# atosystem/SpeechCLIP

Hardware: AMD Instinct MI355X
Metric: speech-image pairs/sec/node (Parallel SpeechCLIP base) (higher is better)
Workload: dtype bf16; 1 GPU; Parallel SpeechCLIP base (HuBERT-base + ViT-B/32) forward + InfoNCE, 10 s/16 kHz audio + 224^2 images; pairs_per_gpu=256, global_batch=256, audio_samples=160000, frames=499, parallelism=single, weights=random-init (no network), mode=forward + loss

## Files before the change

include/speechclip_hip.h:

```cpp
#ifndef SPEECHCLIP_HIP_H
#define SPEECHCLIP_HIP_H

#include <stdint.h>

#ifdef __cplusplus
extern "C" {
#endif

int sc_abi_version(void);
const char* sc_last_error(void);

#define SC_ACT_NONE 0
#define SC_ACT_GELU 1
#define SC_ACT_QUICKGELU 2
#define SC_GEMM_ACT_MASK 0x3
#define SC_GEMM_OUT_F32 0x10
#define SC_GEMM_F16 0x20
#define SC_GEMM_RES_AFTER_ACT 0x0

int sc_gemm_bf16(const void* A, int64_t lda, const void* W, int64_t ldw, void* C, int64_t ldc,
                 const float* bias, const void* residual, int64_t ldr,
                 int64_t M, int N, int K, int flags, void* stream);
int sc_set_gemm_workspace(void* workspace, int64_t bytes);
int sc_gemm_last_path(void);
int sc_debug_vendor_stream_slot(void* stream);

int sc_gemm_bf16_batched(const void* A, int64_t lda, int64_t strideA, const void* W, int64_t ldw,
                         int64_t strideW, int w_mod, void* C, int64_t ldc, int64_t strideC,
                         const float* bias, int64_t M, int N, int K, int batch, int flags, void* stream);
int sc_gemm_bf16_batched2(const void* A, int64_t lda, int64_t strideA, int64_t strideA2, const void* W, int64_t ldw, int64_t strideW, int64_t strideW2,
                          void* C, int64_t ldc, int64_t strideC, int64_t strideC2, int64_t M, int N, int K, int outer, int inner, int flags, void* stream);

#define SC_LN_IN_F32 0x1
#define SC_LN_OUT_F32 0x2
#define SC_LN_GELU 0x4
#define SC_LN_OUT_F16 0x8
int sc_layernorm(const void* x, int64_t ld_in, const float* gamma, const float* beta, void* out, int64_t ld_out,
                 int64_t rows, int D, float eps, int flags, void* stream);

#define SC_WS_NORMALIZE 0x1
#define SC_WS_IN_F32 0x2
int sc_weighted_sum_fwd(const void* hidden, int64_t layer_stride, const float* weights, void* out, int n_layers,
                        int64_t rows, int D, int flags, float eps, void* stream);

#define SC_L2NORM_IN_F32 0x1
#define SC_L2NORM_CLAMP 0x2
int sc_l2norm_fwd(const void* x, int64_t ld_in, float* out, int64_t rows, int D, int flags, void* stream);

int sc_hidden_normalize(void* hidden, int in_f32, int n_layers, int B, int Tp, int T, int D, int method, float* workspace, void* stream);

int sc_splitk_reduce_f32(const float* partials, int nsplit, int64_t M, int N, const float* bias, const float* residual, int64_t ldr, float* out, int act,
                         void* stream);

int sc_wave_layernorm(const float* wav, float* out, const int32_t* lens, int B, int64_t ld, float eps, void* stream);

#define SC_ATTN_CAUSAL 0x1
#define SC_ATTN_F16 0x2
int sc_attention_fwd(const void* q, const void* k, const void* v, void* out, const int32_t* klens, int B, int H,
                     int T, int head_dim, int64_t ld_qkv, int64_t ld_out, float scale, int flags, void* stream);

int sc_attention_fwd_dropout(const void* q, const void* k, const void* v, void* out, const int32_t* klens, int B, int H, int T, int head_dim,
                             int64_t ld_qkv, int64_t ld_out, float scale, int causal, float drop_p, uint32_t seed, void* stream);
int sc_dropout_bf16(const void* x, const void* residual, void* out, int64_t n, float drop_p, uint32_t seed, void* stream);
int sc_dropout_add_layernorm_bf16(const void* x, const void* residual, const float* gamma, const float* beta, void* out, int64_t rows, int D, float eps,
                                  float drop_p, uint32_t seed, void* stream);

int sc_cls_attention_fwd(const void* cls_qkv, const void* kv_x, int64_t ld_kv, const int32_t* lens, void* out, int B, int T,
                         int NQ, int H, int head_dim, float scale, void* stream);

#define SC_ATTN_HD_OUT_F32 0x10
int sc_attention_hd_fwd(const void* q, const void* k, const void* v, void* out, const int32_t* klens, int B, int H, int Tq, int Tk,
                        int head_dim, int64_t q_bs, int64_t q_rs, int64_t kv_bs, int64_t kv_rs, int64_t o_bs, int64_t o_rs,
                        float scale, float drop_p, uint32_t seed, int flags, void* stream);

int sc_attention_rows_fwd(const void* q, const void* k, const void* v, void* out, const uint8_t* key_padding_mask, int B, int H, int L,
                          int head_dim, int64_t ld_qkv, int64_t ld_out, float scale, void* stream);

int sc_attention_probs_fwd(const void* q, const void* k, float* probs, const uint8_t* key_padding_mask, int B, int H, int L, int head_dim,
                           int n_rows, int64_t ld_qkv, float scale, void* stream);

int sc_topk_rows_f32(const float* x, int64_t ld, int64_t rows, int V, int K, float* vals, int32_t* idx, void* stream);

int sc_cls_pool_fwd(const void* x, int64_t ld_x, const void* cls_tok, const float* scores, const float* cls_scores,
                    const int32_t* lens, void* xbar, int B, int T, int NQ, int R, int D, void* stream);
int sc_cls_pool_fwd_split(const void* x, int64_t ld_x, const void* cls_tok, const float* scores, const float* cls_scores,
                          const int32_t* lens, void* xbar_hilo, int B, int T, int NQ, int R, int D, int nblk, void* stream);

int64_t sc_conv0_stats_workspace_bytes(int B);
int sc_conv0_gn_coef(const float* wav, int64_t ld, const float* w, const float* gamma, const float* beta, void* workspace,
                     float* coef, int B, int C, int T0, float eps, void* stream);
int64_t sc_conv0_wfrag_workspace_bytes(int B);
int sc_conv0_fwd(const float* wav, int64_t ld, int64_t L, const float* w, const float* bias, const float* coef, void* out, int B,
                 int C, int T0, int P, int mode, void* wfrag_ws, void* stream);

int sc_posconv_conv(const void* x, const int32_t* valid, const void* wg, void* conv, int B, int Tp, int D, int G, int Kw, void* stream);
int sc_posconv_pack(const void* x, const int32_t* valid, void* xg, int B, int Tp, int D, int G, int Kw, void* stream);
int sc_posconv_finish(const void* x, const int32_t* valid, const void* conv, const float* bias, const float* gamma, const float* beta,
                      void* out, int B, int Tp, int D, int G, int out_f32, float eps, void* stream);

int sc_crop_pad(const float* wav, int64_t ld, const int32_t* starts, const int32_t* lens, float* out, int B, int Lout, void* stream);

int sc_image_normalize_u8(const void* u8_hwc, float* out_chw, int B, int H, int W, const float* mean3, const float* std3, void* stream);
int sc_vit_patchify(const float* img, void* cols, int B, int R, int p, int Kpad, void* stream);
int sc_vit_embed(const void* patch, const float* cls, const float* pos, const float* gamma, const float* beta, float* out, int B,
                 int ntok, int D, float eps, void* stream);

int64_t sc_infonce_workspace_bytes(int Bg);
int sc_infonce_fwd(const float* feat_a, const float* feat_b, const int64_t* ids, void* workspace, float* out3, int Bg, int E,
                   float inv_temperature, float margin, int dcl, int a2b, int b2a, void* stream);

int sc_kw_affine(const float* x, const float* scale, const float* shift, float* out, int64_t rows, int K, int D, void* stream);
int64_t sc_cosine_workspace_bytes(int R, int V);
int sc_cosine_scores(const float* a, const float* emb, void* workspace, float* out, int R, int V, int E, float eps, void* stream);
int sc_cosine_refine(float* scores, const float* a, const float* emb, int R, int V, int E, float delta, float eps, void* stream);
int64_t sc_vq_workspace_bytes(int R, int V);
int sc_vq_fwd(const float* scores, int64_t* targets, float* stats2, float* ent_per_t, void* workspace, int R, int K, int V,
              const int32_t* host_mask_ids, int n_mask, void* stream);
int sc_gather_rows(const float* src, const int64_t* idx, float* out, int R, int E, void* stream);
int sc_retrieval_ranks(const float* score, int64_t ld, const int64_t* own_ids, const int64_t* cand_ids, int32_t* rank, int n, int m, void* stream);

int sc_sgemm(int transa, int transb, int M, int N, int K, float alpha, const float* A, int64_t lda, const float* B, int64_t ldb, float beta,
             float* C, int64_t ldc, const float* bias, void* stream);
int sc_sgemm_batched(int transa, int transb, int M, int N, int K, float alpha, const float* A, int64_t lda, int64_t strideA, const float* B,
                     int64_t ldb, int64_t strideB, float beta, float* C, int64_t ldc, int64_t strideC, const float* bias, int64_t strideBias,
                     int batch, void* stream);
int sc_cls_pool_train_fwd(const void* x, int64_t ld_x, const float* cls_tok, const float* scores, const float* cls_scores,
                          const int32_t* lens, float* p_out, float* xbar, int B, int T, int NQ, int R, int D, float drop_p, uint32_t seed,
                          void* stream);
int sc_cls_pool_bwd(const void* x, int64_t ld_x, const float* cls_tok, const void* hidden, int hidden_f32, int64_t layer_stride, int n_layers,
                    int normalize,
                    const float* p, const float* dzbar, const float* u, const int32_t* lens, float* ds_ws, float* pp_ws, float* du,
                    float* dcls_key, float* dalpha, int B, int T, int NQ, int R, int D, int nsplit, float drop_p, uint32_t seed, void* stream);
int sc_layernorm_bwd(const float* x, const float* dy, const float* gamma, float* dx, float* dgamma, float* dbeta, float* stats_ws, int rows,
                     int D, float eps, int accumulate_dx, void* stream);
int sc_gelu_f32(const float* z, float* y_or_dh, int64_t n, int backward, void* stream);
int sc_colsum(const float* x, int64_t ld, int rows, int cols, float* out, int accumulate, void* stream);
int sc_l2norm_bwd(const float* x, const float* dy, float* dx, int rows, int D, void* stream);
int sc_dropout_f32(const float* x, float* y, int64_t n, float drop_p, uint32_t seed, void* stream);
int sc_add_rows_f32(const float* a, const float* b, float* out, int rows, int cols, int b_rows, float alpha, void* stream);
int sc_mix_softmax_bwd(const float* w, const float* dalpha_b, int B, int n, float* dw, void* stream);
int sc_split_hilo_bf16(const float* a, int64_t lda, void* out, int64_t M, int K, int nblk, void* stream);
int sc_attn_small_bwd(const void* qkv, const float* dout, float* dqkv, int B, int L, int heads, int head_dim, int causal, void* stream);
int sc_quickgelu_f32(const float* z, void* y_or_dh, int64_t n, int backward, int out_bf16, void* stream);
int sc_vq_st_bwd(const float* cos_scores, float* dprob_inout, float* rowdot, int R, int V, float temp, const int* mask_ids, int n_mask, void* stream);
int sc_cosine_bwd_finish(const float* a, const float* G, const float* rowdot, float* da, int R, int E, float eps, void* stream);
int sc_kw_bn_train_fwd(const float* x, const float* gamma, const float* beta, float* y, float* mean_out, float* rstd_out, float* running_mean,
                       float* running_var, int B, int K, int E, float momentum, float eps, void* stream);
int sc_kw_bn_bwd(const float* x, const float* dy, const float* gamma, const float* mean, const float* rstd, float* dx, float* dgamma, float* dbeta,
                 int B, int K, int E, void* stream);
int64_t sc_infonce_bwd_workspace_bytes(int Bg);
int sc_infonce_bwd(const float* feat_a, const float* feat_b, const int64_t* ids, const void* fwd_workspace, void* bwd_workspace, float* G,
// ... 59 lines not shown
```

speechclip_amd/_lib.py:

```python
import ctypes
import os
from ctypes import c_char_p, c_float, c_int, c_int64, c_uint32, c_void_p

import torch

_HERE = os.path.dirname(os.path.abspath(__file__))
LIB_PATH = os.environ.get("SPEECHCLIP_HIP_LIB") or os.path.join(_HERE, "libspeechclip_hip.so")

ACT_NONE, ACT_GELU, ACT_QUICKGELU = 0, 1, 2
GEMM_OUT_F32 = 0x10
GEMM_F16 = 0x20
ATTN_CAUSAL, ATTN_F16 = 0x1, 0x2
ATTN_HD_OUT_F32 = 0x10

_lib = None


class SpeechClipHipError(RuntimeError):
    pass


def lib():
    global _lib
    if _lib is None:
        if not os.path.exists(LIB_PATH):
            raise SpeechClipHipError(
                f"{LIB_PATH} not found: build it with `python -c 'import __graft_entry__ as g; g.build()'` "
                "(make -C speechclip_amd/csrc).  There is no CPU/PyTorch fallback for the hot path.")
        _lib = ctypes.CDLL(LIB_PATH)
        _lib.sc_last_error.restype = c_char_p
        _declare(_lib)
        mode = os.environ.get("SC_GEMM_KERNEL_MODE")
        if mode:
            try:
                _lib.sc_debug_set_gemm_mode(int(mode))
            except ValueError:
                import warnings
                warnings.warn(f"SC_GEMM_KERNEL_MODE={mode!r} is not an integer: ignored")
    return _lib


def _declare(L):
    P, I, L64, F, U32 = c_void_p, c_int, c_int64, c_float, c_uint32
    sigs = {
        "sc_abi_version": ([], c_int),
        "sc_set_gemm_workspace": ([P, L64], c_int),
        "sc_gemm_bf16": ([P, L64, P, L64, P, L64, P, P, L64, L64, I, I, I, P], c_int),
        "sc_gemm_bf16_batched": ([P, L64, L64, P, L64, L64, I, P, L64, L64, P, L64, I, I, I, I, P], c_int),
        "sc_layernorm": ([P, L64, P, P, P, L64, L64, I, F, I, P], c_int),
        "sc_weighted_sum_fwd": ([P, L64, P, P, I, L64, I, I, F, P], c_int),
        "sc_transpose_bf16": ([P, L64, L64, P, L64, L64, I, I, I, I, P], c_int),
        "sc_attn_softmax_bwd": ([P, P, L64, L64, P, L64, P, L64, L64, P, P, P, I, I, I, F, P], c_int),
        "sc_attn_softmax_bwd_dropout": ([P, P, L64, L64, P, L64, P, L64, L64, P, P, P, I, I, I, F, F, U32, I, I, P], c_int),
        "sc_attn_softmax_bwd_heads": ([P, P, L64, L64, P, L64, P, L64, L64, P, P, P, I, I, I, I, F, F, U32, P], c_int),
        "sc_attn_bwd_probs": ([P, P, P, L64, P, P, L64, P, P, P, I, I, I, I, F, F, U32, P], c_int),
        "sc_gemm_bf16_batched2": ([P, L64, L64, L64, P, L64, L64, L64, P, L64, L64, L64, L64, I, I, I, I, I, P], c_int),
        "sc_gelu_bwd_bf16": ([P, P, P, L64, P], c_int),
        "sc_layernorm_bwd_bf16_partials": ([L64], c_int64),
        "sc_layernorm_bwd_bf16": ([P, P, P, P, P, L64, I, F, P], c_int),
        "sc_colsum_bf16_workspace_bytes": ([L64, I], c_int64),
        "sc_colsum_bf16": ([P, L64, L64, I, P, P, I, P], c_int),
        "sc_axpy_bf16": ([P, P, F, L64, P], c_int),
        "sc_cls_pool_dz": ([P, P, P, P, P, P, I, I, I, I, I, L64, P], c_int),
        "sc_l2norm_fwd": ([P, L64, P, L64, I, I, P], c_int),
        "sc_splitk_reduce_f32": ([P, I, L64, I, P, P, L64, P, I, P], c_int),
        "sc_hidden_normalize": ([P, I, I, I, I, I, I, I, P, P], c_int),
        "sc_wave_layernorm": ([P, P, P, I, L64, F, P], c_int),
        "sc_attention_fwd": ([P, P, P, P, P, I, I, I, I, L64, L64, F, I, P], c_int),
        "sc_attention_fwd_dropout": ([P, P, P, P, P, I, I, I, I, L64, L64, F, I, F, U32, P], c_int),
        "sc_attention_hd_fwd": ([P, P, P, P, P, I, I, I, I, I, L64, L64, L64, L64, L64, L64, F, F, U32, I, P], c_int),
        "sc_dropout_bf16": ([P, P, P, L64, F, U32, P], c_int),
        "sc_dropout_add_layernorm_bf16": ([P, P, P, P, P, L64, I, F, F, U32, P], c_int),
        "sc_cls_attention_fwd": ([P, P, L64, P, P, I, I, I, I, I, F, P], c_int),
        "sc_attention_rows_fwd": ([P, P, P, P, P, I, I, I, I, L64, L64, F, P], c_int),
        "sc_attention_probs_fwd": ([P, P, P, P, I, I, I, I, I, L64, F, P], c_int),
        "sc_posconv_finish_train": ([P, P, P, P, P, P, I, I, I, I, P], c_int),
        "sc_posconv_dgrad_finish": ([P, P, P, P, I, I, I, I, P], c_int),
        "sc_reverse_rows_bf16": ([P, P, I, I, I, P], c_int),
        "sc_conv0_bwd": ([P, L64, P, P, P, P, P, I, I, I, I, F, P], c_int),
        "sc_conv0_wgrad": ([P, L64, P, P, I, I, I, I, P], c_int),
        "sc_topk_rows_f32": ([P, L64, L64, I, I, P, P, P], c_int),
        "sc_cls_pool_fwd": ([P, L64, P, P, P, P, P, I, I, I, I, I, P], c_int),
        "sc_cls_pool_fwd_split": ([P, L64, P, P, P, P, P, I, I, I, I, I, I, P], c_int),
        "sc_conv0_stats_workspace_bytes": ([I], c_int64),
        "sc_conv0_gn_coef": ([P, L64, P, P, P, P, P, I, I, I, F, P], c_int),
        "sc_conv0_wfrag_workspace_bytes": ([I], c_int64),
        "sc_conv0_fwd": ([P, L64, L64, P, P, P, P, I, I, I, I, I, P, P], c_int),
        "sc_posconv_conv": ([P, P, P, P, I, I, I, I, I, P], c_int),
        "sc_posconv_pack": ([P, P, P, I, I, I, I, I, P], c_int),
        "sc_posconv_finish": ([P, P, P, P, P, P, P, I, I, I, I, I, F, P], c_int),
        "sc_crop_pad": ([P, L64, P, P, P, I, I, P], c_int),
        "sc_conv0_fwd_packed": ([P, L64, L64, P, P, P, P, I, I, I, P, I, I, I, P, P], c_int),
        "sc_posconv_conv_packed": ([P, P, P, P, P, I, I, I, I, I, P], c_int),
        "sc_posconv_finish_packed": ([P, P, P, P, P, P, P, P, I, L64, I, I, I, F, P], c_int),
        "sc_attention_fwd_packed": ([P, P, P, P, P, P, I, I, I, L64, I, L64, L64, F, F, U32, I, P], c_int),
        "sc_unpack_rows": ([P, L64, P, P, L64, I, I, I, I, I, P], c_int),
        "sc_pack_rows": ([P, L64, P, P, L64, I, I, I, L64, I, I, P], c_int),
        "sc_attention_bwd_packed_workspace_bytes": ([L64, I], c_int64),
        "sc_attention_bwd_packed": ([P, P, P, L64, P, P, L64, P, P, I, I, I, L64, I, F, F, U32, P, P, P, L64, P, P], c_int),
        "sc_image_normalize_u8": ([P, P, I, I, I, P, P, P], c_int),
        "sc_vit_patchify": ([P, P, I, I, I, I, P], c_int),
        "sc_vit_embed": ([P, P, P, P, P, P, I, I, I, F, P], c_int),
        "sc_infonce_workspace_bytes": ([I], c_int64),
        "sc_infonce_fwd": ([P, P, P, P, P, I, I, F, F, I, I, I, P], c_int),
        "sc_kw_affine": ([P, P, P, P, L64, I, I, P], c_int),
        "sc_cosine_workspace_bytes": ([I, I], c_int64),
        "sc_cosine_scores": ([P, P, P, P, I, I, I, F, P], c_int),
        "sc_vq_workspace_bytes": ([I, I], c_int64),
        "sc_vq_fwd": ([P, P, P, P, P, I, I, I, P, I, P], c_int),
        "sc_gather_rows": ([P, P, P, I, I, P], c_int),
        "sc_retrieval_ranks": ([P, L64, P, P, P, I, I, P], c_int),
        "sc_sgemm": ([I, I, I, I, I, F, P, L64, P, L64, F, P, L64, P, P], c_int),
        "sc_sgemm_batched": ([I, I, I, I, I, F, P, L64, L64, P, L64, L64, F, P, L64, L64, P, L64, I, P], c_int),
        "sc_cls_pool_train_fwd": ([P, L64, P, P, P, P, P, P, I, I, I, I, I, F, U32, P], c_int),
        "sc_cls_pool_bwd": ([P, L64, P, P, I, L64, I, I, P, P, P, P, P, P, P, P, P, I, I, I, I, I, I, F, U32, P], c_int),
        "sc_layernorm_bwd": ([P, P, P, P, P, P, P, I, I, F, I, P], c_int),
        "sc_gelu_f32": ([P, P, L64, I, P], c_int),
        "sc_gemm_last_path": ([], c_int),
        "sc_debug_set_gemm_mode": ([I], None),
        "sc_debug_poison_gemm_sched": ([], c_int),
        "sc_debug_vendor_stream_slot": ([P], c_int),
        "sc_split_hilo_bf16": ([P, L64, P, L64, I, I, P], c_int),
        "sc_cosine_refine": ([P, P, P, I, I, I, F, F, P], c_int),
        "sc_attn_small_bwd": ([P, P, P, I, I, I, I, I, P], c_int),
        "sc_quickgelu_f32": ([P, P, L64, I, I, P], c_int),
        "sc_vq_st_bwd": ([P, P, P, I, I, F, P, I, P], c_int),
        "sc_cosine_bwd_finish": ([P, P, P, P, I, I, F, P], c_int),
        "sc_kw_bn_train_fwd": ([P, P, P, P, P, P, P, P, I, I, I, F, F, P], c_int),
        "sc_kw_bn_bwd": ([P, P, P, P, P, P, P, P, I, I, I, P], c_int),
        "sc_colsum": ([P, L64, I, I, P, I, P], c_int),
        "sc_l2norm_bwd": ([P, P, P, I, I, P], c_int),
        "sc_dropout_f32": ([P, P, L64, F, U32, P], c_int),
        "sc_mix_softmax_bwd": ([P, P, I, I, P, P], c_int),
        "sc_add_rows_f32": ([P, P, P, I, I, I, F, P], c_int),
        "sc_infonce_bwd_workspace_bytes": ([I], c_int64),
        "sc_infonce_bwd": ([P, P, P, P, P, P, P, I, I, F, F, I, I, I, P], c_int),
        "sc_grad_norm_workspace_bytes": ([], c_int64),
        "sc_grad_norm": ([P, L64, F, P, P, P], c_int),
        "sc_adam_step": ([P, P, P, P, L64, P, F, F, F, F, F, I, P], c_int),
    }
    for name, (args, res) in sigs.items():
        fn = getattr(L, name)
        fn.argtypes = args
        fn.restype = res


def check(rc, what):
    if rc != 0:
        raise SpeechClipHipError(f"{what} failed (rc={rc}): {lib().sc_last_error().decode()}")


def ptr(t):
    return 0 if t is None else t.data_ptr()


def stream():
# ... 9 lines not shown
```

speechclip_amd/csrc/attention_rows.hip:

```cpp
#include "common.h"
#include "../../include/speechclip_hip.h"

namespace {

constexpr int ROWS_PER_BLOCK = 4;
constexpr int MAX_HD = 1024;

__global__ __launch_bounds__(256) void attention_rows_kernel(const bf16_t* __restrict__ q, const bf16_t* __restrict__ k, const bf16_t* __restrict__ v,
                                                             bf16_t* __restrict__ out, const uint8_t* __restrict__ pad, int B, int H, int L, int hd,
                                                             int64_t ld_qkv, int64_t ld_out, float scale_log2e) {
    extern __shared__ float sq[];
    const int lane = threadIdx.x & 63, wave = threadIdx.x >> 6;
    const int qblocks = (L + ROWS_PER_BLOCK - 1) / ROWS_PER_BLOCK;
    const int bh = blockIdx.x / qblocks, qb = blockIdx.x - bh * qblocks;
    const int b = bh / H, h = bh - b * H;
    const int i = qb * ROWS_PER_BLOCK + wave;
    if (i >= L) return;
    float* myq = sq + wave * hd;
    const bf16_t* qrow = q + ((int64_t)b * L + i) * ld_qkv + h * hd;
    for (int d = lane; d < hd; d += 64) myq[d] = bf2f(qrow[d]) * scale_log2e;
    __builtin_amdgcn_wave_barrier();
    asm volatile("s_waitcnt lgkmcnt(0)" ::: "memory");
    const int nd = (hd + 63) / 64;
    float acc[MAX_HD / 64];
#pragma unroll
    for (int m = 0; m < MAX_HD / 64; ++m) acc[m] = 0.f;
    float run_max = -INFINITY, run_sum = 0.f;
    const uint8_t* prow = pad ? pad + (int64_t)b * L : nullptr;
    for (int j0 = 0; j0 < L; j0 += 64) {
        const int j = j0 + lane;
        const bool valid = j < L && !(prow && prow[j]);
        float s = -INFINITY;
        if (valid) {
            const bf16_t* krow = k + ((int64_t)b * L + j) * ld_qkv + h * hd;
            float dot = 0.f;
            int d = 0;
            for (; d + 8 <= hd; d += 8) {
                const uint4 kk = *(const uint4*)(krow + d);
                dot = fmaf(lo2f(kk.x), myq[d], dot);     dot = fmaf(hi2f(kk.x), myq[d + 1], dot);
                dot = fmaf(lo2f(kk.y), myq[d + 2], dot); dot = fmaf(hi2f(kk.y), myq[d + 3], dot);
                dot = fmaf(lo2f(kk.z), myq[d + 4], dot); dot = fmaf(hi2f(kk.z), myq[d + 5], dot);
                dot = fmaf(lo2f(kk.w), myq[d + 6], dot); dot = fmaf(hi2f(kk.w), myq[d + 7], dot);
            }
            for (; d < hd; ++d) dot = fmaf(bf2f(krow[d]), myq[d], dot);
            s = dot;
        }
        const float cmax = wave_max(s);
        if (cmax == -INFINITY) continue;
        const float nmax = fmaxf(run_max, cmax);
        const float corr = __builtin_amdgcn_exp2f(run_max - nmax);
        const float p = valid ? __builtin_amdgcn_exp2f(s - nmax) : 0.f;
        run_sum = run_sum * corr + wave_sum(p);
        run_max = nmax;
#pragma unroll
        for (int m = 0; m < MAX_HD / 64; ++m)
            if (m < nd) acc[m] *= corr;
        const int jn = L - j0 < 64 ? L - j0 : 64;
        for (int jj = 0; jj < jn; ++jj) {
            const float pj = __shfl(p, jj, 64);
            if (pj == 0.f) continue;
            const bf16_t* vrow = v + ((int64_t)b * L + j0 + jj) * ld_qkv + h * hd;
#pragma unroll
            for (int m = 0; m < MAX_HD / 64; ++m) {
                const int d = lane + 64 * m;
                if (m < nd && d < hd) acc[m] = fmaf(pj, bf2f(vrow[d]), acc[m]);
            }
        }
    }
    const float inv = run_sum > 0.f ? 1.0f / run_sum : 0.f;
    bf16_t* orow = out + ((int64_t)b * L + i) * ld_out + h * hd;
#pragma unroll
    for (int m = 0; m < MAX_HD / 64; ++m) {
        const int d = lane + 64 * m;
        if (m < nd && d < hd) orow[d] = f2bf(acc[m] * inv);
    }
}

}

extern "C" int sc_attention_rows_fwd(const void* q, const void* k, const void* v, void* out, const uint8_t* key_padding_mask, int B, int H, int L,
                                     int head_dim, int64_t ld_qkv, int64_t ld_out, float scale, void* stream) {
    SC_CHECK_ARG(head_dim >= 1 && head_dim <= MAX_HD, "sc_attention_rows_fwd: head_dim=%d must be in [1, %d]", head_dim, MAX_HD);
    SC_CHECK_ARG(head_dim % 8 == 0 && ld_qkv % 8 == 0, "sc_attention_rows_fwd: head_dim and ld_qkv must be multiples of 8 (16-byte key chunks)");
    SC_CHECK_ARG((((uintptr_t)q | (uintptr_t)k | (uintptr_t)v) & 15) == 0, "sc_attention_rows_fwd: q/k/v must be 16-byte aligned");
    SC_CHECK_ARG(q && k && v && out, "sc_attention_rows_fwd: null operand");
    if (B <= 0 || L <= 0 || H <= 0) return 0;
    const int64_t blocks = (int64_t)B * H * ((L + ROWS_PER_BLOCK - 1) / ROWS_PER_BLOCK);
    SC_CHECK_ARG(blocks < 0x7fffffff, "sc_attention_rows_fwd: grid too large");
    hipLaunchKernelGGL(attention_rows_kernel, dim3((unsigned)blocks), dim3(ROWS_PER_BLOCK * 64), ROWS_PER_BLOCK * head_dim * sizeof(float),
                       (hipStream_t)stream, (const bf16_t*)q, (const bf16_t*)k, (const bf16_t*)v, (bf16_t*)out, key_padding_mask, B, H, L, head_dim, ld_qkv,
                       ld_out, scale * 1.44269504088896341f);
    SC_CHECK_LAUNCH();
    return 0;
}
```

speechclip_amd/module/clip_model.py:

```python
from dataclasses import dataclass

import torch
import torch.nn as nn

from .. import ops
from ..ops import ACT_QUICKGELU


@dataclass
class ClipConfig:
    image_resolution: int = 224
    vision_patch: int = 32
    vision_width: int = 768
    vision_layers: int = 12
    embed_dim: int = 512
    context_length: int = 77
    vocab_size: int = 49408
    text_width: int = 512
    text_heads: int = 8
    text_layers: int = 12

    @staticmethod
    def from_name(name: str) -> "ClipConfig":
        if name == "ViT-B/32":
            return ClipConfig()
        if name == "ViT-B/16":
            return ClipConfig(vision_patch=16)
        if name == "ViT-L/14":
            return ClipConfig(vision_patch=14, vision_width=1024, vision_layers=24, embed_dim=768, text_width=768, text_heads=12)
        raise NotImplementedError(f"CLIP variant {name} is not on the MI355X hot path (ViT-B/32, ViT-B/16, ViT-L/14 are)")


class _InProjAttn(nn.Module):
    def __init__(self, d):
        super().__init__()
        self.in_proj_weight = nn.Parameter(torch.empty(3 * d, d))
        self.in_proj_bias = nn.Parameter(torch.zeros(3 * d))
        self.out_proj = nn.Linear(d, d)


class _Mlp(nn.Module):
    def __init__(self, d):
        super().__init__()
        self.c_fc = nn.Linear(d, 4 * d)
        self.c_proj = nn.Linear(4 * d, d)


class _ResBlock(nn.Module):
    def __init__(self, d):
        super().__init__()
        self.attn = _InProjAttn(d)
        self.ln_1 = nn.LayerNorm(d)
        self.mlp = _Mlp(d)
        self.ln_2 = nn.LayerNorm(d)


class _Tower(nn.Module):
    def __init__(self, width, layers, heads):
        super().__init__()
        self.width, self.layers, self.heads = width, layers, heads
        self.resblocks = nn.ModuleList([_ResBlock(width) for _ in range(layers)])
        proj_std = (width ** -0.5) * ((2 * layers) ** -0.5)
        for blk in self.resblocks:
            nn.init.normal_(blk.attn.in_proj_weight, std=width ** -0.5)
            nn.init.normal_(blk.attn.out_proj.weight, std=proj_std)
            nn.init.normal_(blk.mlp.c_fc.weight, std=(2 * width) ** -0.5)
            nn.init.normal_(blk.mlp.c_proj.weight, std=proj_std)

    def pack(self, dev):
        bf, f32 = torch.bfloat16, torch.float32
        out = []
        for b in self.resblocks:
            out.append(dict(
                ln1=(b.ln_1.weight.detach().to(dev, f32), b.ln_1.bias.detach().to(dev, f32)),
                wqkv=b.attn.in_proj_weight.detach().to(dev, bf).contiguous(), bqkv=b.attn.in_proj_bias.detach().to(dev, f32),
                wo=b.attn.out_proj.weight.detach().to(dev, bf).contiguous(), bo=b.attn.out_proj.bias.detach().to(dev, f32),
                ln2=(b.ln_2.weight.detach().to(dev, f32), b.ln_2.bias.detach().to(dev, f32)),
                w1=b.mlp.c_fc.weight.detach().to(dev, bf).contiguous(), b1=b.mlp.c_fc.bias.detach().to(dev, f32),
                w2=b.mlp.c_proj.weight.detach().to(dev, bf).contiguous(), b2=b.mlp.c_proj.bias.detach().to(dev, f32)))
        return out


def run_tower(packed, x, B, L, heads, causal=False):
    M, W = x.shape
    dev = x.device
    bf = torch.bfloat16
    n = torch.empty(M, W, device=dev, dtype=bf)
    qkv = torch.empty(M, 3 * W, device=dev, dtype=bf)
    att = torch.empty(M, W, device=dev, dtype=bf)
    ffn = torch.empty(M, 4 * W, device=dev, dtype=bf)
    for L_ in packed:
        ops.layernorm(x, *L_["ln1"], out=n)
        ops.gemm(n, L_["wqkv"], L_["bqkv"], out=qkv)
        ops.attention(qkv, B, L, heads, None, out=att, causal=causal)
        ops.gemm(att, L_["wo"], L_["bo"], residual=x, out=x, out_f32=True)
        ops.layernorm(x, *L_["ln2"], out=n)
        ops.gemm(n, L_["w1"], L_["b1"], ACT_QUICKGELU, out=ffn)
        ops.gemm(ffn, L_["w2"], L_["b2"], residual=x, out=x, out_f32=True)
    return x


class _Visual(nn.Module):
    def __init__(self, cfg: ClipConfig):
        super().__init__()
        w, p, r = cfg.vision_width, cfg.vision_patch, cfg.image_resolution
        self.input_resolution, self.output_dim, self.patch = r, cfg.embed_dim, p
        self.conv1 = nn.Conv2d(3, w, kernel_size=p, stride=p, bias=False)
        scale = w ** -0.5
        self.class_embedding = nn.Parameter(scale * torch.randn(w))
        self.positional_embedding = nn.Parameter(scale * torch.randn((r // p) ** 2 + 1, w))
        self.ln_pre = nn.LayerNorm(w)
        self.transformer = _Tower(w, cfg.vision_layers, max(1, w // 64))
        self.ln_post = nn.LayerNorm(w)
        self.proj = nn.Parameter(scale * torch.randn(w, cfg.embed_dim))


class CLIP(nn.Module):

    def __init__(self, cfg: ClipConfig):
        super().__init__()
        self.cfg = cfg
        self.context_length = cfg.context_length
        self.visual = _Visual(cfg)
        self.transformer = _Tower(cfg.text_width, cfg.text_layers, cfg.text_heads)
        self.vocab_size = cfg.vocab_size
        self.token_embedding = nn.Embedding(cfg.vocab_size, cfg.text_width)
        self.positional_embedding = nn.Parameter(torch.empty(cfg.context_length, cfg.text_width))
        self.ln_final = nn.LayerNorm(cfg.text_width)
        self.text_projection = nn.Parameter(torch.empty(cfg.text_width, cfg.embed_dim))
        self.logit_scale = nn.Parameter(torch.ones([]) * 2.6592600)
        nn.init.normal_(self.token_embedding.weight, std=0.02)
        nn.init.normal_(self.positional_embedding, std=0.01)
        nn.init.normal_(self.text_projection, std=cfg.text_width ** -0.5)
        self._packed = None
        self._packed_bwd = None
        self.register_load_state_dict_post_hook(lambda module, keys: module.invalidate_packed())

    def invalidate_packed(self):
        self._packed = None
        self._packed_bwd = None

    def packed_bwd(self, dev):
        if getattr(self, "_packed_bwd", None) is None:
            f32, bf = torch.float32, torch.bfloat16
            c = lambda t: t.detach().to(dev, f32).contiguous()
            def t16(t):
                wt = t.detach().to(dev, f32).t().contiguous().to(bf)
                return torch.cat([wt, wt], dim=1).contiguous()

            self._packed_bwd = dict(
                txt=[dict(g1=c(b.ln_1.weight), wqkvt=t16(b.attn.in_proj_weight), wot=t16(b.attn.out_proj.weight), g2=c(b.ln_2.weight),
                          w1t=t16(b.mlp.c_fc.weight), w2t=t16(b.mlp.c_proj.weight)) for b in self.transformer.resblocks],
                ln_final_g=c(self.ln_final.weight), txt_proj=t16(self.text_projection.t()))
        return self._packed_bwd

    def _apply(self, fn, *a, **k):
        self._packed = None
        self._packed_bwd = None
        return super()._apply(fn, *a, **k)

    @property
    def dtype(self):
        return self.visual.conv1.weight.dtype

    def _pack(self, dev):
        bf, f32 = torch.bfloat16, torch.float32
        v, cfg = self.visual, self.cfg
        K = 3 * v.patch * v.patch
        Kpad = (K + 63) // 64 * 64
        w = torch.zeros(cfg.vision_width, Kpad, device=dev, dtype=bf)
        w[:, :K] = v.conv1.weight.detach().reshape(cfg.vision_width, K).to(dev, bf)
        P = dict(Kpad=Kpad, conv_w=w, cls=v.class_embedding.detach().to(dev, f32), pos=v.positional_embedding.detach().to(dev, f32).contiguous(),
                 ln_pre=(v.ln_pre.weight.detach().to(dev, f32), v.ln_pre.bias.detach().to(dev, f32)),
                 ln_post=(v.ln_post.weight.detach().to(dev, f32), v.ln_post.bias.detach().to(dev, f32)),
                 proj_t=v.proj.detach().t().to(dev, bf).contiguous(), vis=v.transformer.pack(dev),
                 txt=self.transformer.pack(dev), txt_pos=self.positional_embedding.detach().to(dev, f32).contiguous(),
                 ln_final=(self.ln_final.weight.detach().to(dev, f32), self.ln_final.bias.detach().to(dev, f32)),
                 txt_proj_t=self.text_projection.detach().t().to(dev, bf).contiguous())
        return P

    def packed(self, dev):
        if self._packed is None:
            self._packed = self._pack(dev)
        return self._packed

    @torch.no_grad()
    def encode_image(self, image: torch.Tensor) -> torch.Tensor:
        assert image.is_cuda, "CLIP.encode_image runs on the HIP kernels only (no CPU fallback)"
        v = self.visual
        P = self.packed(image.device)
        B = image.shape[0]
        ntok = (v.input_resolution // v.patch) ** 2 + 1
        W = self.cfg.vision_width
        cols = ops.vit_patchify(image.float().contiguous(), v.patch, P["Kpad"])
        patch = ops.gemm(cols, P["conv_w"])
        x = ops.vit_embed(patch, P["cls"], P["pos"], *P["ln_pre"], B, ntok, W)
        run_tower(P["vis"], x, B, ntok, v.transformer.heads)
        cls = ops.layernorm(x, *P["ln_post"], rows=B, D=W, ld_in=ntok * W)
        return ops.gemm(cls, P["proj_t"], out_f32=True)

    def encode_text_embeddings(self, emb: torch.Tensor, take_pos) -> torch.Tensor:
        assert emb.is_cuda
        if torch.is_grad_enabled() and emb.requires_grad:
            from ..train_tail import TextTowerTrainFn
            if not isinstance(take_pos, int):
                pos = int(take_pos[0].item())
                assert bool((take_pos == pos).all()), "training path: one EOT position for the whole batch (K keywords => K + 1)"
                take_pos = pos
            return TextTowerTrainFn.apply(self, emb, take_pos)
        with torch.no_grad():
            return self._encode_text_embeddings_eval(emb, take_pos)

    def _encode_text_embeddings_eval(self, emb: torch.Tensor, take_pos: torch.Tensor) -> torch.Tensor:
        P = self.packed(emb.device)
        B, L, tw = emb.shape
        x = (emb.float() + P["txt_pos"][:L]).reshape(B * L, tw).contiguous()
        run_tower(P["txt"], x, B, L, self.transformer.heads, causal=True)
        if isinstance(take_pos, int):
            rows = x.view(B, L, tw)[:, take_pos].contiguous()
        else:
            rows = x.view(B, L, tw)[torch.arange(B, device=emb.device), take_pos].contiguous()
        n = ops.layernorm(rows, *P["ln_final"])
        return ops.gemm(n, P["txt_proj_t"], out_f32=True)
```

speechclip_amd/ops.py:

```python
from typing import Optional

import torch

from . import _lib
from ._lib import ACT_GELU, ACT_NONE, ACT_QUICKGELU, ATTN_CAUSAL, ATTN_F16, ATTN_HD_OUT_F32, GEMM_F16, GEMM_OUT_F32, check, lib, ptr, stream

bf16 = torch.bfloat16

PROFILE = None
PROFILE_HBM = None


class _HbmSpan:
    __slots__ = ("tag", "nbytes", "e0")

    def __init__(self, tag, nbytes):
        self.tag, self.nbytes, self.e0 = tag, nbytes, None

    def __enter__(self):
        if PROFILE_HBM is not None:
            self.e0 = torch.cuda.Event(enable_timing=True)
            self.e0.record()
        return self

# ... 213 lines not shown
    _need_cuda(x, residual)
    assert x.dtype == bf16 and residual.dtype == bf16 and x.is_contiguous() and residual.is_contiguous() and x.shape == residual.shape and x.dim() == 2
    if out is None:
        out = torch.empty_like(x)
    rc = lib().sc_dropout_add_layernorm_bf16(ptr(x), ptr(residual), ptr(gamma), ptr(beta), ptr(out), x.shape[0], x.shape[1], eps, float(drop_p),
                                             int(seed) & 0xffffffff, stream())
    if rc == 1:
        dropout_bf16(x, drop_p, seed, residual=residual, out=x)
        return layernorm(x, gamma, beta, eps, out=out)
    check(rc, "sc_dropout_add_layernorm_bf16")
    return out


ATTN_HD_DIMS = (64, 96, 128)


def attention_hd(q, k, v, B, H, Tq, Tk, hd, q_strides, kv_strides, klens_i32=None, out=None, out_f32=False, scale=None, drop_p=0.0, seed=0):
    _need_cuda(q, k, v)
    assert q.dtype == bf16 and k.dtype == bf16 and v.dtype == bf16
    D = H * hd
    if out is None:
        out = torch.empty(B, Tq, D, device=q.device, dtype=torch.float32 if out_f32 else bf16)
    assert out.dtype == (torch.float32 if out_f32 else bf16) and out.is_contiguous() and out.numel() == B * Tq * D
    check(lib().sc_attention_hd_fwd(ptr(q), ptr(k), ptr(v), ptr(out), ptr(klens_i32), B, H, Tq, Tk, hd, q_strides[0], q_strides[1],
                                    kv_strides[0], kv_strides[1], Tq * D, D, hd ** -0.5 if scale is None else scale, float(drop_p),
                                    int(seed) & 0xffffffff, ATTN_HD_OUT_F32 if out_f32 else 0, stream()), "sc_attention_hd_fwd")
    return out


def attention_hd_qkv(qkv, B, L, H, klens_i32=None, out_f32=False, drop_p=0.0, seed=0):
    assert qkv.dim() == 2 and qkv.is_contiguous() and qkv.shape[0] == B * L and qkv.shape[1] % (3 * H) == 0
    D = qkv.shape[1] // 3
    s = (L * 3 * D, 3 * D)
    out = attention_hd(qkv, qkv[:, D:], qkv[:, 2 * D:], B, H, L, L, D // H, s, s, klens_i32, out_f32=out_f32, drop_p=drop_p, seed=seed)
    return out.view(B * L, D)


def attention_rows(qkv, B, L, H, hd, key_padding_mask=None, scale=None):
    _need_cuda(qkv, key_padding_mask)
    D = H * hd
    assert qkv.dtype == bf16 and qkv.shape == (B * L, 3 * D) and qkv.is_contiguous()
    m = None
    if key_padding_mask is not None:
        assert key_padding_mask.shape == (B, L)
        m = key_padding_mask.to(torch.uint8).contiguous()
    out = torch.empty(B * L, D, device=qkv.device, dtype=bf16)
    check(lib().sc_attention_rows_fwd(qkv.data_ptr(), qkv.data_ptr() + D * 2, qkv.data_ptr() + 2 * D * 2, ptr(out), ptr(m), B, H, L, hd, 3 * D, D,
                                      hd ** -0.5 if scale is None else scale, stream()), "sc_attention_rows_fwd")
    return out


def attention_probs(qkv, B, L, H, hd, key_padding_mask=None, n_rows=None, scale=None):
    _need_cuda(qkv, key_padding_mask)
    D = H * hd
    assert qkv.dtype == bf16 and qkv.shape == (B * L, 3 * D) and qkv.is_contiguous()
    n_rows = L if n_rows is None else int(n_rows)
    m = None
    if key_padding_mask is not None:
        assert key_padding_mask.shape == (B, L)
        m = key_padding_mask.to(torch.uint8).contiguous()
    probs = torch.empty(B, H, n_rows, L, device=qkv.device, dtype=torch.float32)
    check(lib().sc_attention_probs_fwd(qkv.data_ptr(), qkv.data_ptr() + D * 2, ptr(probs), ptr(m), B, H, L, hd, n_rows, 3 * D,
                                       hd ** -0.5 if scale is None else scale, stream()), "sc_attention_probs_fwd")
    return probs


def topk_rows(x, k):
    _need_cuda(x)
    x2 = x.float().contiguous().view(-1, x.shape[-1])
    R, V = x2.shape
    vals = torch.empty(R, k, device=x.device, dtype=torch.float32)
    idx = torch.empty(R, k, device=x.device, dtype=torch.int32)
    check(lib().sc_topk_rows_f32(ptr(x2), V, R, V, int(k), ptr(vals), ptr(idx), stream()), "sc_topk_rows_f32")
    return vals.view(*x.shape[:-1], k), idx.long().view(*x.shape[:-1], k)


def cls_attention(cls_qkv, kv_x, lens_i32, B, T, NQ, H, hd):
    _need_cuda(cls_qkv, kv_x)
    D = H * hd
    assert cls_qkv.shape == (NQ, 3 * D) and kv_x.shape == (B * T, 2 * D) and cls_qkv.is_contiguous() and kv_x.is_contiguous()
    out = torch.empty(B, NQ, D, device=kv_x.device, dtype=bf16)
    check(lib().sc_cls_attention_fwd(ptr(cls_qkv), ptr(kv_x), 2 * D, ptr(lens_i32), ptr(out), B, T, NQ, H, hd, hd ** -0.5, stream()),
          "sc_cls_attention_fwd")
    return out


def cls_pool(x_rows, cls16, scores, cls_scores, lens_i32, B, T, NQ, R, D, split=0):
    _need_cuda(x_rows, cls16, scores, cls_scores)
    assert x_rows.dtype == bf16 and x_rows.stride(1) == 1 and scores.dtype == torch.float32 and scores.shape == (B * T, R) and scores.is_contiguous()
    xbar = torch.empty(B, R, (split or 1) * D, device=x_rows.device, dtype=bf16)
    if split:
        check(lib().sc_cls_pool_fwd_split(ptr(x_rows), x_rows.stride(0), ptr(cls16), ptr(scores), ptr(cls_scores), ptr(lens_i32), ptr(xbar), B, T, NQ, R, D,
                                          int(split), stream()), "sc_cls_pool_fwd_split")
    else:
        check(lib().sc_cls_pool_fwd(ptr(x_rows), x_rows.stride(0), ptr(cls16), ptr(scores), ptr(cls_scores), ptr(lens_i32), ptr(xbar), B, T, NQ, R, D,
                                    stream()), "sc_cls_pool_fwd")
    return xbar


def conv0(wav, w, T0, P, gn_gamma=None, gn_beta=None, bias=None, eps=1e-5, out=None, ln_coef=None):
    _need_cuda(wav, w)
    B, L = wav.shape
    C = w.shape[0]
    assert wav.dtype == torch.float32 and wav.is_contiguous() and w.dtype == torch.float32 and w.is_contiguous()
    buf = out if out is not None else torch.zeros(B * P + 8, C, device=wav.device, dtype=bf16)
    assert buf.dtype == bf16 and buf.is_contiguous() and buf.shape[0] >= B * P and buf.shape[1] == C
    wfrag = torch.empty(lib().sc_conv0_wfrag_workspace_bytes(B), device=wav.device, dtype=torch.uint8)
    if gn_gamma is not None:
        ws = torch.empty(lib().sc_conv0_stats_workspace_bytes(B), device=wav.device, dtype=torch.uint8)
        coef = torch.empty(B, C, 2, device=wav.device, dtype=torch.float32)
        with _HbmSpan("conv0_gn_stats", B * L * 4):
            check(lib().sc_conv0_gn_coef(ptr(wav), L, ptr(w), ptr(gn_gamma), ptr(gn_beta), ptr(ws), ptr(coef), B, C, T0, eps, stream()), "sc_conv0_gn_coef")
        with _HbmSpan("conv0", B * L * 4 + B * P * C * 2):
            check(lib().sc_conv0_fwd(ptr(wav), L, L, ptr(w), None, ptr(coef), ptr(buf), B, C, T0, P, 0, ptr(wfrag), stream()), "sc_conv0_fwd")
    else:
        assert ln_coef is None or (ln_coef.dtype == torch.float32 and ln_coef.numel() == 2 * C + 1 and ln_coef.is_contiguous())
        with _HbmSpan("conv0", B * L * 4 + B * P * C * 2):
            check(lib().sc_conv0_fwd(ptr(wav), L, L, ptr(w), ptr(bias), ptr(ln_coef), ptr(buf), B, C, T0, P, 1 if ln_coef is None else 2, ptr(wfrag), stream()), "sc_conv0_fwd")
    return buf


def posconv(x, valid_i32, wg, bias, gamma, beta, B, Tp, D, G, Kw, out=None, out_f32=False, eps=1e-5):
    _need_cuda(x, wg)
    cg = D // G
    conv = torch.empty(B * G * Tp * cg, device=x.device, dtype=bf16)
    rc = lib().sc_posconv_conv(ptr(x), ptr(valid_i32), ptr(wg), ptr(conv), B, Tp, D, G, Kw, stream())
    if rc == 1:
        xg = torch.empty(B * G * (Tp + Kw) * cg + 64, device=x.device, dtype=bf16)
        check(lib().sc_posconv_pack(ptr(x), ptr(valid_i32), ptr(xg), B, Tp, D, G, Kw, stream()), "sc_posconv_pack")
        gemm_batched(xg, cg, (Tp + Kw) * cg, wg, cg * Kw * cg, G, conv, cg, Tp * cg, None, Tp, cg, Kw * cg, B * G)
    else:
        check(rc, "sc_posconv_conv")
    if out is None:
        out = torch.empty(B * Tp, D, device=x.device, dtype=torch.float32 if out_f32 else bf16)
    check(lib().sc_posconv_finish(ptr(x), ptr(valid_i32), ptr(conv), ptr(bias), ptr(gamma), ptr(beta), ptr(out), B, Tp, D, G,
                                  int(out.dtype == torch.float32), eps, stream()), "sc_posconv_finish")
    return out


def conv0_packed(wav, w, T0, row_off_i32, row_scale, rows_max, total_rows, gn_gamma=None, gn_beta=None, bias=None, eps=1e-5, out=None, ln_coef=None):
    _need_cuda(wav, w, row_off_i32)
    B, L = wav.shape
    C = w.shape[0]
    assert wav.dtype == torch.float32 and wav.is_contiguous() and w.dtype == torch.float32 and w.is_contiguous() and row_off_i32.dtype == torch.int32
    assert out is not None and out.dtype == bf16 and out.is_contiguous() and out.shape[0] >= row_scale * total_rows and out.shape[1] == C
    wfrag = torch.empty(lib().sc_conv0_wfrag_workspace_bytes(B), device=wav.device, dtype=torch.uint8)
    coef = None
    if gn_gamma is not None:
        ws = torch.empty(lib().sc_conv0_stats_workspace_bytes(B), device=wav.device, dtype=torch.uint8)
        coef = torch.empty(B, C, 2, device=wav.device, dtype=torch.float32)
        with _HbmSpan("conv0_gn_stats", B * L * 4):
            check(lib().sc_conv0_gn_coef(ptr(wav), L, ptr(w), ptr(gn_gamma), ptr(gn_beta), ptr(ws), ptr(coef), B, C, T0, eps, stream()), "sc_conv0_gn_coef")
    mode = 0 if gn_gamma is not None else 1
    if ln_coef is not None:
        assert gn_gamma is None and ln_coef.dtype == torch.float32 and ln_coef.numel() == 2 * C + 1 and ln_coef.is_contiguous()
        coef, mode = ln_coef, 2
    with _HbmSpan("conv0", row_scale * total_rows * (5 * 4 + C * 2)):
        check(lib().sc_conv0_fwd_packed(ptr(wav), L, L, ptr(w), None if gn_gamma is not None else ptr(bias), ptr(coef), ptr(out), B, C, T0,
                                        ptr(row_off_i32), row_scale, row_scale * rows_max, mode, ptr(wfrag), stream()),
              "sc_conv0_fwd_packed")
    return out


def posconv_packed(x, valid_i32, row_off_i32, wg, bias, gamma, beta, B, rows_max, total_rows, D, G, Kw, out=None, out_f32=False, eps=1e-5):
    _need_cuda(x, wg, row_off_i32)
    cg = D // G
# ... 625 lines not shown
```

Before: 6241 pairs/s.

## Compute only the CLS row in the last ViT block

```diff
diff --git a/include/speechclip_hip.h b/include/speechclip_hip.h
--- a/include/speechclip_hip.h
+++ b/include/speechclip_hip.h
@@ -67,6 +67,9 @@
 
 int sc_cls_attention_fwd(const void* cls_qkv, const void* kv_x, int64_t ld_kv, const int32_t* lens, void* out, int B, int T,
                          int NQ, int H, int head_dim, float scale, void* stream);
+
+int sc_vit_cls_attention(const void* q, int64_t ld_q, const void* kv, int64_t ld_kv, void* out, int64_t ld_out, const int32_t* klens, int B, int H,
+                         int T, int head_dim, float scale, int flags, void* stream);
 
 #define SC_ATTN_HD_OUT_F32 0x10
 int sc_attention_hd_fwd(const void* q, const void* k, const void* v, void* out, const int32_t* klens, int B, int H, int Tq, int Tk,
diff --git a/speechclip_amd/_lib.py b/speechclip_amd/_lib.py
--- a/speechclip_amd/_lib.py
+++ b/speechclip_amd/_lib.py
@@ -72,6 +72,7 @@
         "sc_dropout_bf16": ([P, P, P, L64, F, U32, P], c_int),
         "sc_dropout_add_layernorm_bf16": ([P, P, P, P, P, L64, I, F, F, U32, P], c_int),
         "sc_cls_attention_fwd": ([P, P, L64, P, P, I, I, I, I, I, F, P], c_int),
+        "sc_vit_cls_attention": ([P, L64, P, L64, P, L64, P, I, I, I, I, F, I, P], c_int),
         "sc_attention_rows_fwd": ([P, P, P, P, P, I, I, I, I, L64, L64, F, P], c_int),
         "sc_attention_probs_fwd": ([P, P, P, P, I, I, I, I, I, L64, F, P], c_int),
         "sc_posconv_finish_train": ([P, P, P, P, P, P, I, I, I, I, P], c_int),
diff --git a/speechclip_amd/csrc/attention_rows.hip b/speechclip_amd/csrc/attention_rows.hip
--- a/speechclip_amd/csrc/attention_rows.hip
+++ b/speechclip_amd/csrc/attention_rows.hip
@@ -76,6 +76,86 @@
     }
 }
 
+
+constexpr int CLS_WAVES = 4;
+
+template <bool F16> __device__ __forceinline__ float x2f(bf16_t v) {
+    if constexpr (F16) return (float)__builtin_bit_cast(_Float16, v); else return bf2f(v);
+}
+
+template <bool F16>
+__global__ __launch_bounds__(CLS_WAVES * 64) void vit_cls_attention_kernel(const bf16_t* __restrict__ q, int64_t ld_q, const bf16_t* __restrict__ kv, int64_t ld_kv,
+                                                                           bf16_t* __restrict__ out, int64_t ld_out, const int32_t* __restrict__ klens, int BH, int H,
+                                                                           int T, float scale_log2e) {
+    __shared__ float sq[CLS_WAVES][64];
+    const int lane = threadIdx.x & 63, wave = threadIdx.x >> 6;
+    const int bh = blockIdx.x * CLS_WAVES + wave;
+    if (bh >= BH) return;
+    const int b = bh / H, h = bh - b * H;
+    int n = klens ? klens[b] : T;
+    n = n < 0 ? 0 : (n > T ? T : n);
+    float* myq = sq[wave];
+    myq[lane] = x2f<F16>(q[(int64_t)b * ld_q + h * 64 + lane]) * scale_log2e;
+    __builtin_amdgcn_wave_barrier();
+    asm volatile("s_waitcnt lgkmcnt(0)" ::: "memory");
+    const bf16_t* kbase = kv + (int64_t)b * T * ld_kv + h * 64;
+    const bf16_t* vbase = kbase + H * 64;
+    const int g = lane >> 3, c8 = (lane & 7) * 8;
+    float acc[8];
+#pragma unroll
+    for (int e = 0; e < 8; ++e) acc[e] = 0.f;
+    float run_max = -INFINITY, run_sum = 0.f;
+    for (int j0 = 0; j0 < n; j0 += 64) {
+        const int j = j0 + lane;
+        float s = -INFINITY;
+        if (j < n) {
+            const bf16_t* krow = kbase + (int64_t)j * ld_kv;
+            float dot = 0.f;
+#pragma unroll
+            for (int d = 0; d < 64; d += 8) {
+                const uint4 kk = *(const uint4*)(krow + d);
+                dot = fmaf(lo2fx<F16>(kk.x), myq[d], dot);     dot = fmaf(hi2fx<F16>(kk.x), myq[d + 1], dot);
+                dot = fmaf(lo2fx<F16>(kk.y), myq[d + 2], dot); dot = fmaf(hi2fx<F16>(kk.y), myq[d + 3], dot);
+                dot = fmaf(lo2fx<F16>(kk.z), myq[d + 4], dot); dot = fmaf(hi2fx<F16>(kk.z), myq[d + 5], dot);
+                dot = fmaf(lo2fx<F16>(kk.w), myq[d + 6], dot); dot = fmaf(hi2fx<F16>(kk.w), myq[d + 7], dot);
+            }
+            s = dot;
+        }
+        const float nmax = fmaxf(run_max, wave_max(s));
+        const float corr = __builtin_amdgcn_exp2f(run_max - nmax);
+        const float p = j < n ? __builtin_amdgcn_exp2f(s - nmax) : 0.f;
+        run_sum = run_sum * corr + wave_sum(p);
+        run_max = nmax;
+#pragma unroll
+        for (int e = 0; e < 8; ++e) acc[e] *= corr;
+#pragma unroll
+        for (int i = 0; i < 8; ++i) {
+            const int jj = g + 8 * i;
+            const float pj = __shfl(p, jj, 64);
+            if (j0 + jj < n) {
+                const uint4 vv = *(const uint4*)(vbase + (int64_t)(j0 + jj) * ld_kv + c8);
+                acc[0] = fmaf(pj, lo2fx<F16>(vv.x), acc[0]); acc[1] = fmaf(pj, hi2fx<F16>(vv.x), acc[1]);
+                acc[2] = fmaf(pj, lo2fx<F16>(vv.y), acc[2]); acc[3] = fmaf(pj, hi2fx<F16>(vv.y), acc[3]);
+                acc[4] = fmaf(pj, lo2fx<F16>(vv.z), acc[4]); acc[5] = fmaf(pj, hi2fx<F16>(vv.z), acc[5]);
+                acc[6] = fmaf(pj, lo2fx<F16>(vv.w), acc[6]); acc[7] = fmaf(pj, hi2fx<F16>(vv.w), acc[7]);
+            }
+        }
+    }
+#pragma unroll
+    for (int e = 0; e < 8; ++e) {
+        acc[e] += __shfl_xor(acc[e], 8, 64);
+        acc[e] += __shfl_xor(acc[e], 16, 64);
+        acc[e] += __shfl_xor(acc[e], 32, 64);
+    }
+    if (g == 0) {
+        const float inv = run_sum > 0.f ? 1.0f / run_sum : 0.f;
+        uint4 o;
+        o.x = pack2x<F16>(acc[0] * inv, acc[1] * inv); o.y = pack2x<F16>(acc[2] * inv, acc[3] * inv);
+        o.z = pack2x<F16>(acc[4] * inv, acc[5] * inv); o.w = pack2x<F16>(acc[6] * inv, acc[7] * inv);
+        *(uint4*)(out + (int64_t)b * ld_out + h * 64 + c8) = o;
+    }
+}
+
 }
 
 extern "C" int sc_attention_rows_fwd(const void* q, const void* k, const void* v, void* out, const uint8_t* key_padding_mask, int B, int H, int L,
@@ -93,3 +173,28 @@
     SC_CHECK_LAUNCH();
     return 0;
 }
+
+extern "C" int sc_vit_cls_attention(const void* q, int64_t ld_q, const void* kv, int64_t ld_kv, void* out, int64_t ld_out, const int32_t* klens, int B, int H,
+                                    int T, int head_dim, float scale, int flags, void* stream) {
+    SC_CHECK_ARG(head_dim == 64, "sc_vit_cls_attention: head_dim=%d (64 only: the CLIP towers)", head_dim);
+    SC_CHECK_ARG(q && kv && out, "sc_vit_cls_attention: null operand");
+    SC_CHECK_ARG((flags & ~SC_ATTN_F16) == 0, "sc_vit_cls_attention: flags=%d (SC_ATTN_F16 only)", flags);
+    if (B <= 0 || H <= 0) return 0;
+    SC_CHECK_ARG(T >= 1, "sc_vit_cls_attention: T=%d", T);
+    SC_CHECK_ARG(ld_q >= (int64_t)H * 64 && ld_kv >= (int64_t)2 * H * 64 && ld_out >= (int64_t)H * 64,
+                 "sc_vit_cls_attention: ld_q / ld_out must cover H * 64 columns and ld_kv 2 * H * 64 (k | v)");
+    SC_CHECK_ARG(ld_kv % 8 == 0 && ld_out % 8 == 0, "sc_vit_cls_attention: ld_kv and ld_out must be multiples of 8 (16-byte pieces)");
+    SC_CHECK_ARG((((uintptr_t)kv | (uintptr_t)out) & 15) == 0, "sc_vit_cls_attention: kv / out must be 16-byte aligned");
+    const int64_t bh = (int64_t)B * H;
+    SC_CHECK_ARG(bh < 0x7fffffff, "sc_vit_cls_attention: grid too large");
+    const dim3 grid((unsigned)((bh + CLS_WAVES - 1) / CLS_WAVES)), block(CLS_WAVES * 64);
+    const float sl2 = scale * 1.44269504088896341f;
+    if (flags & SC_ATTN_F16)
+        hipLaunchKernelGGL(vit_cls_attention_kernel<true>, grid, block, 0, (hipStream_t)stream, (const bf16_t*)q, ld_q, (const bf16_t*)kv, ld_kv, (bf16_t*)out, ld_out,
+                           klens, (int)bh, H, T, sl2);
+    else
+        hipLaunchKernelGGL(vit_cls_attention_kernel<false>, grid, block, 0, (hipStream_t)stream, (const bf16_t*)q, ld_q, (const bf16_t*)kv, ld_kv, (bf16_t*)out, ld_out,
+                           klens, (int)bh, H, T, sl2);
+    SC_CHECK_LAUNCH();
+    return 0;
+}
diff --git a/speechclip_amd/module/clip_model.py b/speechclip_amd/module/clip_model.py
--- a/speechclip_amd/module/clip_model.py
+++ b/speechclip_amd/module/clip_model.py
@@ -1,3 +1,4 @@
+import os
 from dataclasses import dataclass
 
 import torch
@@ -78,10 +79,17 @@
                 ln2=(b.ln_2.weight.detach().to(dev, f32), b.ln_2.bias.detach().to(dev, f32)),
                 w1=b.mlp.c_fc.weight.detach().to(dev, bf).contiguous(), b1=b.mlp.c_fc.bias.detach().to(dev, f32),
                 w2=b.mlp.c_proj.weight.detach().to(dev, bf).contiguous(), b2=b.mlp.c_proj.bias.detach().to(dev, f32)))
+        W = self.width
+        for d in out:
+            d.update(wq=d["wqkv"][:W], bq=d["bqkv"][:W], wkv=d["wqkv"][W:], bkv=d["bqkv"][W:])
         return out
 
 
-def run_tower(packed, x, B, L, heads, causal=False):
+def vit_last_cls_enabled() -> bool:
+    return os.environ.get("SC_VIT_LAST_CLS", "1") != "0"
+
+
+def run_tower(packed, x, B, L, heads, causal=False, last_cls=False):
     M, W = x.shape
     dev = x.device
     bf = torch.bfloat16
@@ -89,7 +97,8 @@
     qkv = torch.empty(M, 3 * W, device=dev, dtype=bf)
     att = torch.empty(M, W, device=dev, dtype=bf)
     ffn = torch.empty(M, 4 * W, device=dev, dtype=bf)
-    for L_ in packed:
+    full = packed[:-1] if last_cls and not causal else packed
+    for L_ in full:
         ops.layernorm(x, *L_["ln1"], out=n)
         ops.gemm(n, L_["wqkv"], L_["bqkv"], out=qkv)
         ops.attention(qkv, B, L, heads, None, out=att, causal=causal)
@@ -97,7 +106,23 @@
         ops.layernorm(x, *L_["ln2"], out=n)
         ops.gemm(n, L_["w1"], L_["b1"], ACT_QUICKGELU, out=ffn)
         ops.gemm(ffn, L_["w2"], L_["b2"], residual=x, out=x, out_f32=True)
+    if len(full) < len(packed):
+        _last_block_cls(packed[-1], x, n, qkv, B, L, heads)
     return x
+
+
+def _last_block_cls(L_, x, n, qkv, B, L, heads):
+    M, W = x.shape
+    ops.layernorm(x, *L_["ln1"], out=n)
+    kv = qkv.view(-1)[:M * 2 * W].view(M, 2 * W)
+    ops.gemm(n, L_["wkv"], L_["bkv"], out=kv)
+    q = ops.gemm(n, L_["wq"], L_["bq"], M=B, K=W, lda=L * W)
+    att = ops.vit_cls_attention(q, kv, B, L, heads)
+    xc = x.view(B, L * W)[:, :W]
+    ops.gemm(att, L_["wo"], L_["bo"], residual=xc, out=xc, out_f32=True)
+    n2 = ops.layernorm(x, *L_["ln2"], rows=B, D=W, ld_in=L * W)
+    ffn = ops.gemm(n2, L_["w1"], L_["b1"], ACT_QUICKGELU)
+    ops.gemm(ffn, L_["w2"], L_["b2"], residual=xc, out=xc, out_f32=True)
 
 
 class _Visual(nn.Module):
@@ -184,20 +209,29 @@
             self._packed = self._pack(dev)
         return self._packed
 
-    @torch.no_grad()
-    def encode_image(self, image: torch.Tensor) -> torch.Tensor:
+    def _image_tokens(self, image: torch.Tensor):
         assert image.is_cuda, "CLIP.encode_image runs on the HIP kernels only (no CPU fallback)"
         v = self.visual
         P = self.packed(image.device)
         B = image.shape[0]
         ntok = (v.input_resolution // v.patch) ** 2 + 1
-        W = self.cfg.vision_width
         cols = ops.vit_patchify(image.float().contiguous(), v.patch, P["Kpad"])
         patch = ops.gemm(cols, P["conv_w"])
-        x = ops.vit_embed(patch, P["cls"], P["pos"], *P["ln_pre"], B, ntok, W)
-        run_tower(P["vis"], x, B, ntok, v.transformer.heads)
+        return ops.vit_embed(patch, P["cls"], P["pos"], *P["ln_pre"], B, ntok, self.cfg.vision_width), B, ntok
+
+    @torch.no_grad()
+    def encode_image(self, image: torch.Tensor) -> torch.Tensor:
+        x, B, ntok = self._image_tokens(image)
+        P, W = self.packed(image.device), self.cfg.vision_width
+        run_tower(P["vis"], x, B, ntok, self.visual.transformer.heads, last_cls=vit_last_cls_enabled())
         cls = ops.layernorm(x, *P["ln_post"], rows=B, D=W, ld_in=ntok * W)
         return ops.gemm(cls, P["proj_t"], out_f32=True)
+
+    @torch.no_grad()
+    def encode_image_tokens(self, image: torch.Tensor) -> torch.Tensor:
+        x, B, ntok = self._image_tokens(image)
+        run_tower(self.packed(image.device)["vis"], x, B, ntok, self.visual.transformer.heads)
+        return x.view(B, ntok, self.cfg.vision_width)
 
     def encode_text_embeddings(self, emb: torch.Tensor, take_pos) -> torch.Tensor:
         assert emb.is_cuda
diff --git a/speechclip_amd/ops.py b/speechclip_amd/ops.py
--- a/speechclip_amd/ops.py
+++ b/speechclip_amd/ops.py
@@ -319,6 +319,19 @@
     out = torch.empty(B, NQ, D, device=kv_x.device, dtype=bf16)
     check(lib().sc_cls_attention_fwd(ptr(cls_qkv), ptr(kv_x), 2 * D, ptr(lens_i32), ptr(out), B, T, NQ, H, hd, hd ** -0.5, stream()),
           "sc_cls_attention_fwd")
+    return out
+
+
+def vit_cls_attention(q, kv, B, T, H, klens_i32=None, out=None, scale=None):
+    _need_cuda(q, kv)
+    D = H * 64
+    assert q.dtype in (bf16, torch.float16) and kv.dtype == q.dtype and q.shape == (B, D) and kv.shape == (B * T, 2 * D) and q.stride(1) == 1 and kv.stride(1) == 1
+    if out is None:
+        out = torch.empty(B, D, device=q.device, dtype=q.dtype)
+    assert out.dtype == q.dtype and out.shape == (B, D) and out.stride(1) == 1
+    assert klens_i32 is None or (klens_i32.dtype == torch.int32 and klens_i32.numel() == B and klens_i32.is_contiguous())
+    check(lib().sc_vit_cls_attention(ptr(q), q.stride(0), ptr(kv), kv.stride(0), ptr(out), out.stride(0), ptr(klens_i32), B, H, T, 64,
+                                     0.125 if scale is None else scale, ATTN_F16 if q.dtype == torch.float16 else 0, stream()), "sc_vit_cls_attention")
     return out
 
 
```

Measured after the change: 6257 pairs/s, median of 6. Within noise of the previous version (+0.3%).
